# miniufo/xinvert

Measured on AMD Instinct MI355X. Metric: SOR grid-points*iters/sec (fp64) at 3600x1800, masked points counted, higher is better.
Workload: dtype f64

## Files before the change

### xinvert_amd/csrc/xinv_pipe2d.h

```cpp
#pragma once
#include "xinv_fused.h"

#define XINV_PIPE_P 4
#ifndef XINV_PIPE_B
#define XINV_PIPE_B 2
#endif
#define XINV_PIPE_LAG (XINV_PIPE_B + 5)
#define XINV_PIPE_NS 4
#define XINV_PIPE_UW(np) (128 * (np) - 4 * XINV_PIPE_P)
#ifndef XINV_PIPE_PF0
#define XINV_PIPE_PF0 4
#endif
#ifndef XINV_PIPE_PF
#define XINV_PIPE_PF 4
#endif

template <class M, unsigned UM> struct PipeRec {
    static constexpr int NCO = M::NC - 1;
    static constexpr int NUNI = __builtin_popcount(UM & ((1u << NCO) - 1u));
    static constexpr bool HOIST = M::template hoist<UM>();
    static constexpr int NW = NUNI + (HOIST ? 2 : 0);
    static constexpr int RW = NW == 0 ? 0 : (NW <= 4 ? 4 : 8);
};

struct RowFactorArgs {
    const double *c[5];
    int64_t sc[5];
    int64_t yc, xc;
    int gen;
    unsigned um;
    int hoist, rw;
    XinvScal sc_;
    double *rowf;
};

#ifdef XINV_AUX_KERNELS
__global__ __launch_bounds__(256) void k_row_factor(RowFactorArgs a)
{
    const int64_t j = (int64_t)blockIdx.x * 256 + threadIdx.x, m = blockIdx.y;
    if (j >= a.yc) return;
    const double u = a.sc_.undef;
    const bool inner = (j >= 1 && j <= a.yc - 2);
    const int nco = a.gen ? 5 : 2;
    const double ones = __longlong_as_double(-1LL);
    double *f = a.rowf + (m * a.yc + j) * a.rw;
    double v[5];
    int k = 0;
    bool def = true;
    for (int q = 0; q < nco; q++) {
        v[q] = 0.0;
        if ((a.um >> q) & 1u) { v[q] = a.c[q][m * a.sc[q] + j * a.xc]; f[k++] = v[q]; def = def && (v[q] != u); }
    }
    if (a.hoist) {
        double rq = 0.0, rok = 0.0;
        if (inner) {
            if (!a.gen) {
                const double aP = a.c[0][m * a.sc[0] + (j + 1) * a.xc], a0 = v[0], c = v[1];
                rq = a.sc_.optArg / ((aP + a0) * a.sc_.ratioSqr + (c + c));
                rok = (def && (aP != u)) ? ones : 0.0;
            } else {
                const double A = v[0], C = v[1], F = v[4];
                rq = a.sc_.optArg / ((A * a.sc_.ratioSqr + C) * 2.0
                                     - F * a.sc_.delxSqr);
                rok = def ? ones : 0.0;
            }
        }
        f[k++] = rq; f[k++] = rok;
    }
    for (; k < a.rw; k++) f[k] = 0.0;
}
#endif

struct PointFactorArgs {
    const double *c[6];
    int64_t sc[6];
    int64_t yc, xc, n;
    XinvScal sc_;
    double *q;
    int *flag;
};
#ifdef XINV_AUX_KERNELS
__global__ __launch_bounds__(256) void k_point_factor(PointFactorArgs a)
{
    const int64_t m = blockIdx.y;
    const double u = a.sc_.undef;
    bool zero = false, differ = false;
    for (int64_t t = (int64_t)blockIdx.x * 256 + threadIdx.x; t < a.n; t += (int64_t)gridDim.x * 256) {
        const int64_t j = t / a.xc;
        const double A = a.c[0][m * a.sc[0] + t], C = a.c[1][m * a.sc[1] + t], Dd = a.c[2][m * a.sc[2] + t];
        const double E = a.c[3][m * a.sc[3] + t], F = a.c[4][m * a.sc[4] + t], G = a.c[5][m * a.sc[5] + t];
        differ = differ || (__double_as_longlong(A) != __double_as_longlong(C));
        const bool ok = (j >= 1) && (j <= a.yc - 2) && (G != u) && (A != u) && (C != u) && (Dd != u) && (E != u) && (F != u);
        double q = 0.0;
        if (ok) {
            q = a.sc_.optArg / ((A * a.sc_.ratioSqr + C) * 2.0
                                - F * a.sc_.delxSqr);
            zero = zero || (q == 0.0);
        }
        a.q[m * a.n + t] = q;
    }
    if (__any(zero) && (threadIdx.x & 63) == 0) atomicOr(a.flag, 1);
    if (__any(differ) && (threadIdx.x & 63) == 0) atomicOr(a.flag, 2);
}
#endif

__device__ __forceinline__ void xinv_pipe_barrier()
{
    asm volatile("s_waitcnt lgkmcnt(0)\n\ts_barrier" ::: "memory");
}

typedef const double __attribute__((address_space(4))) *xinv_cdouble_ptr;
typedef const char __attribute__((address_space(1))) *xinv_gcptr;
typedef char __attribute__((address_space(1))) *xinv_gptr;
typedef double xinv_v2d __attribute__((ext_vector_type(2)));
typedef const xinv_v2d __attribute__((address_space(1))) *xinv_gcd2ptr;
typedef const double __attribute__((address_space(1))) *xinv_gcdptr;
typedef xinv_v2d __attribute__((address_space(1))) *xinv_gd2ptr;
typedef double __attribute__((address_space(1))) *xinv_gdptr;

__device__ __forceinline__ void pipe_extend_fix(double2 &edge, const double2 &inner, double inner_w,
                                                const LaneCols &lc, bool tall, double u)
{
    if (lc.cls_x == 1) { if (inner.x != u) edge.x = inner.x; }
    else if (lc.cls_x == 2) { if (inner.y != u) edge.x = inner.y; }
    else if (lc.cls_x == 3) {
        if (tall && inner.x != u) edge.x = inner.x;
        if (inner_w != u) edge.x = inner_w;
    }
    if (lc.cls_y == 1) { if (inner.y != u) edge.y = inner.y; }
    else if (lc.cls_y == 3) {
        if (tall && inner.y != u) edge.y = inner.y;
        if (inner.x != u) edge.y = inner.x;
    }
}

template <class M, unsigned UM, bool FR, int NP, bool AL, bool EXT, int PW, int PF, bool SEAM = false>
__device__ __forceinline__ void xinv_pipe_wave(const FusedArgs &a, int64_t m, int yu0, int yu1,
                                               const LaneCols (&lc)[NP], const int64_t (&st0)[NP], int lane,
                                               double2 (*ring)[XINV_PIPE_NS][NP * (FR ? 2 : 1)][XINV_WAVE], int gtot,
                                               double &acc, int &cnt,
                                               unsigned long long seam_lanes = 0ull)
{
    constexpr int P = XINV_PIPE_P, H = 2 * P, D = 4, LAG = XINV_PIPE_LAG, B = XINV_PIPE_B;
    constexpr int R = PF + D;
    constexpr int PFR = M::PIPE_PFR;
    using REC = PipeRec<M, UM>;
    constexpr int NC = M::NC, FQ = M::NC - 1, RW = REC::RW;
    constexpr bool HOIST = REC::HOIST;
    constexpr int RS = FR ? 2 : 1;
    static_assert(R % D == 0 && R % B == 0 && R % XINV_PIPE_NS == 0,
                  "the unroll period must keep row parity, ring slots and barriers compile-time");
    const int ycr = (int)a.yc;
    const unsigned rowbytes = (unsigned)a.xc * 8u;
    const double u = a.sc_.undef;
    const int slice_bytes = (int)(rowbytes * (unsigned)ycr);
    const __amdgpu_buffer_rsrc_t rsS = __builtin_amdgcn_make_buffer_rsrc((void *)(a.src + m * a.sS), 0, slice_bytes, 0x00020000);
    const __amdgpu_buffer_rsrc_t rsD = __builtin_amdgcn_make_buffer_rsrc((void *)(a.dst + m * a.sS), 0, slice_bytes, 0x00020000);
    __amdgpu_buffer_rsrc_t rsC[NC];
#pragma unroll
    for (int q = 0; q < NC; q++)
        rsC[q] = __builtin_amdgcn_make_buffer_rsrc((void *)(a.c[q] + m * a.sc[q]), 0, slice_bytes, 0x00020000);
    const xinv_cdouble_ptr rowf = (xinv_cdouble_ptr)(uintptr_t)(reinterpret_cast<const double *>(a.rowf) + m * a.yc * RW);
    unsigned lo0[NP], lo1[NP], so0[NP], so1[NP];
#pragma unroll
    for (int q = 0; q < NP; q++) {
        lo0[q] = (unsigned)lc[q].l0 * 8u; lo1[q] = (unsigned)lc[q].l1 * 8u;
        so0[q] = lc[q].use_x ? (unsigned)st0[q] * 8u : 0xffffffffu;
        so1[q] = lc[q].use_y ? (unsigned)(st0[q] + 1) * 8u : 0xffffffffu;
    }

    unsigned long long okx64[NP], oky64[NP];
    double nsx[NP], nsy[NP];
    int nnx[NP], nny[NP];
#pragma unroll
    for (int q = 0; q < NP; q++) {
        okx64[q] = __builtin_amdgcn_ballot_w64(lc[q].ok_x) & ~seam_lanes; oky64[q] = __builtin_amdgcn_ballot_w64(lc[q].ok_y);
        nsx[q] = nsy[q] = 0.0; nnx[q] = nny[q] = 0;
    }
    static_assert(!SEAM || (NP == 1 && !AL && PipeRec<M, UM>::HOIST),
                  "seam variants: one column pair per lane, per-row records, updates under EXEC masks");

    const int in_lo = yu0 - H + 2 * PW;
    const int in_hi = yu1 - 1 + H - 2 * PW;

    double2 sw[NP][R];
    CoefWin<NC, R> cw[NP];
    double rokw[R];
#pragma unroll
    for (int t = 0; t < R; t++) {
        rokw[t] = 0.0;
#pragma unroll
        for (int q = 0; q < NP; q++) {
            sw[q][t] = make_double2(0.0, 0.0);
            cw[q].rq[t] = 0.0; cw[q].mx[t] = 0u; cw[q].my[t] = 0u;
#pragma unroll
            for (int c = 0; c < NC; c++) { cw[q].v[c][t] = make_double2(0.0, 0.0); cw[q].s[c][t] = 0.0; }
        }
    }

    const int maxo = (int)(rowbytes * (unsigned)(ycr - 1));
    int nxo = (yu0 - H + 2 * PW) * (int)rowbytes;
    int nxr = (yu0 - H + 2 * PW) * (RW * 8);
    auto ldrow = [&](__amdgpu_buffer_rsrc_t rs, int soff, auto qtag) {
        constexpr int q = decltype(qtag)::value;
        double2 v;
        if (AL) {
            const auto t = __builtin_amdgcn_raw_buffer_load_b128(rs, (int)lo0[q], soff, 0);
            v.x = __hiloint2double((int)t[1], (int)t[0]); v.y = __hiloint2double((int)t[3], (int)t[2]);
        } else {
            const auto t0 = __builtin_amdgcn_raw_buffer_load_b64(rs, (int)lo0[q], soff, 0);
            const auto t1 = __builtin_amdgcn_raw_buffer_load_b64(rs, (int)lo1[q], soff, 0);
            v.x = __hiloint2double((int)t0[1], (int)t0[0]); v.y = __hiloint2double((int)t1[1], (int)t1[0]);
        }
        return v;
    };
    auto request = [&](int, auto stag) {
        constexpr int slot = decltype(stag)::value;
        const int soff = min(max(nxo, 0), maxo);
        nxo += (int)rowbytes;
        asm("" : "+s"(nxo));
        xinv_unroll_steps([&](auto qtag) {
            constexpr int q = decltype(qtag)::value;
            if (PW == 0) sw[q][slot] = ldrow(rsS, soff, qtag);
            xinv_unroll_steps([&](auto ctag) {
                constexpr int c = decltype(ctag)::value;
                if (!((UM >> c) & 1u) && !(FR && c == FQ && PW > 0)) cw[q].v[c][slot] = ldrow(rsC[c], soff, qtag);
            }, std::make_integer_sequence<int, NC>{});
        }, std::make_integer_sequence<int, NP>{});
    };
    auto request_rf = [&](int, auto stag) {
        constexpr int slot = decltype(stag)::value;
        if constexpr (RW > 0) {
            const unsigned roff = (unsigned)min(max(nxr, 0), (ycr - 1) * (RW * 8));
            nxr += RW * 8;
            const xinv_cdouble_ptr pr = (xinv_cdouble_ptr)((const char __attribute__((address_space(4))) *)rowf + roff);
            double rec[RW];
#pragma unroll
            for (int k = 0; k < RW; k++) rec[k] = pr[k];
#pragma unroll
            for (int q = 0; q < NP; q++) {
                int k = 0;
#pragma unroll
                for (int c = 0; c < NC - 1; c++)
                    if ((UM >> c) & 1u) cw[q].s[c][slot] = rec[k++];
                if (HOIST) { cw[q].rq[slot] = rec[k]; rokw[slot] = rec[k + 1]; }
            }
        }
    };
    xinv_unroll_steps([&](auto ttag) { request(in_lo + decltype(ttag)::value, ttag); asm volatile("" ::: "memory"); },
                      std::make_integer_sequence<int, PF>{});
    xinv_unroll_steps([&](auto ttag) { request_rf(in_lo + decltype(ttag)::value, ttag); },
                      std::make_integer_sequence<int, PFR>{});

    auto half_pass = [&](auto xtag, auto jtag, auto ptag, auto mtag, auto fixt) {
        constexpr int X = decltype(xtag)::value, sj = decltype(jtag)::value, sjp = decltype(ptag)::value,
                      sjm = decltype(mtag)::value;
        constexpr bool FIX = decltype(fixt)::value;
        static_assert(!FIX || (X == 0 && NP == 1), "column xc-1 sits in an .x slot");
        const double edge = (X == 0) ? xinv_lane_up(sw[NP - 1][sj].y) : xinv_lane_down(sw[0][sj].x);
        double nv[NP];
#pragma unroll
        for (int q = 0; q < NP; q++) {
            double w, e;
            if (X == 0) { w = (q == 0) ? edge : sw[q > 0 ? q - 1 : 0][sj].y; e = sw[q][sj].y; }
            else        { w = sw[q][sj].x; e = (q == NP - 1) ? edge : sw[q < NP - 1 ? q + 1 : q][sj].x; }
            if constexpr (FIX) e = xinv_lane_down(sw[q][sj].x);
            const double t = M::template inc<X, UM, R, false>(cw[q], sj, sjp, comp<X>(sw[q][sj]), comp<X>(sw[q][sjp]),
                                              comp<X>(sw[q][sjm]), w, e, a.sc_);
            if constexpr (HOIST) {
                const unsigned long long rm = (FIX ? seam_lanes : (X ? oky64[q] : okx64[q])) &
                                              (unsigned long long)__double_as_longlong(rokw[sj]);
                if constexpr (ModelFma<M>::value)
                    nv[q] = xinv_fma_where_ne(comp<X>(sw[q][sj]), t, cw[q].rq[sj], comp<X>(cw[q].v[FQ][sj]), u, rm);
                else
                    nv[q] = xinv_add_where_ne(comp<X>(sw[q][sj]), t, comp<X>(cw[q].v[FQ][sj]), u, rm);
            } else {
                const unsigned long long pm = __builtin_amdgcn_ballot_w64((X ? cw[q].my[sj] : cw[q].mx[sj]) != 0u);
                nv[q] = xinv_add_where(comp<X>(sw[q][sj]), t, pm);
            }
        }
#pragma unroll
        for (int q = 0; q < NP; q++) setc<X>(sw[q][sj], nv[q]);
    };
    auto half_sweep = [&](auto xtag, auto jtag, auto ptag, auto mtag) {
        constexpr int X = decltype(xtag)::value;
        half_pass(xtag, jtag, ptag, mtag, std::false_type{});
        if constexpr (SEAM && X == 0) {
            constexpr int sj = decltype(jtag)::value;
            half_pass(xtag, jtag, ptag, mtag, std::true_type{});
            sw[0][sj].y = xinv_bitsel64(seam_lanes, sw[0][sj].x, sw[0][sj].y);
        }
    };

    int g = 0;
#pragma unroll
    for (; g < LAG * PW; g++) {
        if (PW > 0 && g == LAG * PW - 1) {
#pragma unroll
            for (int q = 0; q < NP; q++) {
                sw[q][0] = ring[PW - 1][(2 * PW) % XINV_PIPE_NS][q * RS][lane];
                if (FR) cw[q].v[FQ][0] = ring[PW - 1][(2 * PW) % XINV_PIPE_NS][q * RS + 1][lane];
            }
        }
        if ((g + 1) % B == 0) xinv_pipe_barrier();
    }

    for (int rb_ = in_lo; rb_ <= in_hi; rb_ += R) {
        xinv_unroll_steps([&](auto utag) {
            constexpr int U = decltype(utag)::value;
            constexpr int X = (U & 1) ? 0 : 1;
#define SLOT(w) ((U - (w) + 4 * R) % R)
#define RSLOT(w) ((2 * PW + U - (w) + 64 * XINV_PIPE_NS) % XINV_PIPE_NS)
#define ITAG(v) std::integral_constant<int, (v)>{}
            const int r = rb_ + U;
            request(r + PF, ITAG((U + PF) % R));
            request_rf(r + PFR, ITAG((U + PFR) % R));
            if (PW > 0) {
#pragma unroll
                for (int q = 0; q < NP; q++) {
                    sw[q][(U + 1) % R] = ring[PW - 1][RSLOT(-1)][q * RS][lane];
                    if (FR) cw[q].v[FQ][(U + 1) % R] = ring[PW - 1][RSLOT(-1)][q * RS + 1][lane];
                }
            }
            if constexpr (!HOIST) {
                const bool rv = (r - 1 >= 1) && (r - 1 <= ycr - 2);
#pragma unroll
                for (int q = 0; q < NP; q++)
                    M::template derive<UM, R, false>(cw[q], SLOT(0), SLOT(1), rv && lc[q].ok_x, rv && lc[q].ok_y, a.sc_);
            }
            {
                const int ja = r - 1;
                constexpr int sj = SLOT(1), sjp = SLOT(0), sjm = SLOT(2);
                if (EXT) {
                    if (ja == 1 || ja == ycr - 2) {
                        const double wl = xinv_lane_up(sw[NP - 1][sj].y);
#pragma unroll
                        for (int q = 0; q < NP; q++) {
                            const double iw = (q == 0) ? wl : sw[q > 0 ? q - 1 : 0][sj].y;
                            if (ja == 1) pipe_extend_fix(sw[q][sjm], sw[q][sj], iw, lc[q], a.tall, u);
                            if (ja == ycr - 2) pipe_extend_fix(sw[q][sjp], sw[q][sj], iw, lc[q], a.tall, u);
                        }
                    }
                }
                half_sweep(ITAG(X), ITAG(sj), ITAG(sjp), ITAG(sjm));
            }
            {
                const int jb = r - 2;
                constexpr int sj = SLOT(2), sjp = SLOT(1), sjm = SLOT(3);
                half_sweep(ITAG(X), ITAG(sj), ITAG(sjp), ITAG(sjm));
                if ((unsigned)(jb - yu0) < (unsigned)(yu1 - yu0)) {
#pragma unroll
                    for (int q = 0; q < NP; q++) {
                        const double2 t = sw[q][sj];
                        xinv_norm_row(nsx[q], nsy[q], nnx[q], nny[q], t.x, t.y, u);
                    }
                }
                if (PW < P - 1) {
#pragma unroll
                    for (int q = 0; q < NP; q++) {
                        ring[PW][RSLOT(2)][q * RS][lane] = sw[q][sj];
                        if (FR) ring[PW][RSLOT(2)][q * RS + 1][lane] = cw[q].v[FQ][sj];
                    }
                } else if ((unsigned)(jb - yu0) < (unsigned)(yu1 - yu0)) {
                    const int doff = jb * (int)rowbytes;
                    xinv_unroll_steps([&](auto qtag) {
                        constexpr int q = decltype(qtag)::value;
                        const double2 t = sw[q][sj];
                        typedef unsigned xinv_v4u __attribute__((__vector_size__(16)));
                        typedef unsigned xinv_v2u __attribute__((__vector_size__(8)));
                        if (AL) {
                            const xinv_v4u tv = {(unsigned)__double2loint(t.x), (unsigned)__double2hiint(t.x),
                                                 (unsigned)__double2loint(t.y), (unsigned)__double2hiint(t.y)};
                            __builtin_amdgcn_raw_buffer_store_b128(tv, rsD, (int)so0[q], doff, 0);
                        } else {
                            const xinv_v2u tx = {(unsigned)__double2loint(t.x), (unsigned)__double2hiint(t.x)};
                            const xinv_v2u ty = {(unsigned)__double2loint(t.y), (unsigned)__double2hiint(t.y)};
                            __builtin_amdgcn_raw_buffer_store_b64(tx, rsD, (int)so0[q], doff, 0);
                            __builtin_amdgcn_raw_buffer_store_b64(ty, rsD, (int)so1[q], doff, 0);
                        }
                    }, std::make_integer_sequence<int, NP>{});
                }
            }
            if ((LAG * PW + U + 1) % B == 0) xinv_pipe_barrier();
#undef SLOT
#undef RSLOT
#undef ITAG
        }, std::make_integer_sequence<int, R>{});
        g += R;
    }
    for (; g < gtot; g++) if ((g + 1) % B == 0) xinv_pipe_barrier();
#pragma unroll
    for (int q = 0; q < NP; q++) {
        acc += (lc[q].use_x ? nsx[q] : 0.0);
        acc += (lc[q].use_y ? nsy[q] : 0.0);
        cnt += (lc[q].use_x ? nnx[q] : 0) + (lc[q].use_y ? nny[q] : 0);
    }
}

template <class M, unsigned UM, bool FR, int NP, bool AL, bool EXT, bool SEAM = false>
__global__ __launch_bounds__(64 * XINV_PIPE_P) void k_pipe2d(FusedArgs a_)
{
    xinv_fresh_scalar_cache();
    constexpr int P = XINV_PIPE_P, K = P, H = 2 * K, LAG = XINV_PIPE_LAG, B = XINV_PIPE_B;
    __shared__ double2 ring[P - 1][XINV_PIPE_NS][NP * (FR ? 2 : 1)][XINV_WAVE];

    unsigned tag;
    int T;
    double acc = 0.0;
    int cnt = 0;
    const int wave = threadIdx.x >> 6, lane = threadIdx.x & 63;
    int pwi;
    {
    const FusedArgs &a = a_;
    const int64_t m = a.member0 + blockIdx.y;
    XinvCtl *ctl = a.ctl + m;
    if (!a.force && xinv_ctl_done(ctl)) return;
    if (a.lag && (int)blockIdx.x == a.nwg) { xinv_lag_reduce_prev(a, ctl, m); return; }
    tag = a.lag ? a.tag : xinv_ctl_seq(ctl);

    const int NB = a.nwg;
    {
        const int L = blockIdx.x, q = NB >> 3, rem = NB & 7, xcd = L & 7, idx = L >> 3;
        T = xcd * q + (xcd < rem ? xcd : rem) + idx;
    }
    pwi = (wave + (int)(blockIdx.x >> 8)) & (P - 1);
    int wt = T;
    bool active = wt < a.nstrip * a.nrb;
    if constexpr (SEAM) {
        if (!a.tile_list && NB == a.nstrip * a.nrb)
            wt = xinv_seam_tile(xinv_heavy_first((int)blockIdx.x, NB, (a.nstrip == 1 ? 1 : 2) * a.nrb), a.nstrip, a.nrb);
    }
    if (a.tile_list) {
        wt = a.tile_list[m * a.ntl + T];
        active = wt >= 0;
        wt = active ? wt : 0;
    }
    int rb = wt / a.nstrip, strip = wt - rb * a.nstrip;
    const int64_t xc = a.xc, yc = a.yc;
    int yu0, yu1;
    if (a.RY > 0) {
        yu0 = rb * a.RY;
        yu1 = (yu0 + a.RY < (int)yc) ? yu0 + a.RY : (int)yc;
    } else {
        yu0 = (int)((((int64_t)rb * yc) / a.nrb) & ~(int64_t)1);
        yu1 = (rb + 1 == a.nrb) ? (int)yc : (int)((((int64_t)(rb + 1) * yc) / a.nrb) & ~(int64_t)1);
    }
    const int UW = SEAM ? xinv_ring_uw(xc, H) : XINV_PIPE_UW(NP), HW = SEAM ? xinv_ring_hw(xc, H, strip) : H;
    const int64_t xu0 = (int64_t)strip * UW;
    LaneCols lc[NP];
    int64_t st0[NP];
    RingSeam rs = {0ull, false};
#pragma unroll
    for (int q = 0; q < NP; q++) {
        if constexpr (SEAM) lc[q] = make_lanecols_ring(xu0, HW, UW, lane, xc, rs);
        else lc[q] = make_lanecols<AL>(xu0, H, UW, lane, xc, a.per != 0, NP, q);
        st0[q] = xu0 - HW + 2 * NP * lane + 2 * q;
    }

    if (active) {
        const int ry = yu1 - yu0;
        int gtot = 0;
#pragma unroll
        for (int pw = 0; pw < P; pw++) {
            const int per = (pw == 0 ? XINV_PIPE_PF0 : XINV_PIPE_PF) + 4;
            const int n = ry + 2 * H - 4 * pw;
            const int g = LAG * pw + ((n + per - 1) / per) * per;
            gtot = g > gtot ? g : gtot;
        }
        gtot = ((gtot + B - 1) / B) * B;
        const bool wraps = rs.any;
#define XINV_PIPE_MARCH(SM) \
        switch (pwi) { \
        case 0: xinv_pipe_wave<M, UM, FR, NP, AL, EXT, 0, XINV_PIPE_PF0, SM>(a, m, yu0, yu1, lc, st0, lane, ring, gtot, acc, cnt, rs.lanes); break; \
        case 1: xinv_pipe_wave<M, UM, FR, NP, AL, EXT, 1, XINV_PIPE_PF, SM>(a, m, yu0, yu1, lc, st0, lane, ring, gtot, acc, cnt, rs.lanes); break; \
        case 2: xinv_pipe_wave<M, UM, FR, NP, AL, EXT, 2, XINV_PIPE_PF, SM>(a, m, yu0, yu1, lc, st0, lane, ring, gtot, acc, cnt, rs.lanes); break; \
        default: xinv_pipe_wave<M, UM, FR, NP, AL, EXT, 3, XINV_PIPE_PF, SM>(a, m, yu0, yu1, lc, st0, lane, ring, gtot, acc, cnt, rs.lanes); break; \
        }
        if (wraps) { XINV_PIPE_MARCH(SEAM) } else { XINV_PIPE_MARCH(false) }
#undef XINV_PIPE_MARCH
    }
    }
    const FusedArgs __attribute__((address_space(4))) *kp =
        (const FusedArgs __attribute__((address_space(4))) *)__builtin_amdgcn_kernarg_segment_ptr();
    asm volatile("" : "+s"(kp) :: "memory");
    if (kp->no_ctl) return;
    const int64_t m = kp->member0 + blockIdx.y;
    XinvCtl *ctl = kp->ctl + m;
    const int NB = kp->nwg;
    struct { unsigned long long *psum; const double *xsum; const long long *xcnt; int lag; XinvStop stop; const void *hook; } a;
    a.psum = kp->psum; a.xsum = kp->xsum; a.xcnt = kp->xcnt; a.lag = kp->lag;
    a.hook = XINV_TEST_HOOKS ? (const void *)kp->dbg : nullptr;
    a.stop.mxLoop = kp->stop.mxLoop; a.stop.tolerance = kp->stop.tolerance;
    a.stop.stop_on_zero_norm = kp->stop.stop_on_zero_norm;

    {
        unsigned long long *pw = a.psum + (size_t)m * XINV_KMAX * NB * XINV_PW;
        const double ws = xinv_wave_sum(acc);
        const long long wc = xinv_wave_sum_ll((long long)cnt);
        if (lane == 0 && !xinv_hook_withhold(a.hook, T, tag, m)) {
            const unsigned long long hi = (unsigned long long)tag << 32;
            const unsigned long long bits = (unsigned long long)__double_as_longlong(ws);
            unsigned long long *q = pw + ((size_t)pwi * NB + T) * XINV_PW;
            __hip_atomic_store(q + 0, hi | (bits & 0xffffffffull), __ATOMIC_RELAXED, __HIP_MEMORY_SCOPE_AGENT);
            __hip_atomic_store(q + 1, hi | (bits >> 32), __ATOMIC_RELAXED, __HIP_MEMORY_SCOPE_AGENT);
            __hip_atomic_store(q + 2, hi | (unsigned long long)(unsigned)wc, __ATOMIC_RELAXED,
                               __HIP_MEMORY_SCOPE_AGENT);
        }
        if (a.lag || blockIdx.x != gridDim.x - 1) return;
        __syncthreads();
        xinv_norm_reduce<K, P>(wave, lane, NB, tag, pw, ctl, a.stop, a.xsum ? a.xsum[m] : 0.0,
                               a.xcnt ? a.xcnt[m] : 0);
    }
}
```

### xinvert_amd/csrc/xinv_tiles.h

```cpp
#pragma once
#include <cstdint>
#ifndef __HIPCC__
#ifndef __host__
#define __host__
#endif
#ifndef __device__
#define __device__
#endif
#endif

struct TileRows { int strip; int64_t y0, y1; };
__host__ __device__ inline TileRows xinv_tile_rows(int wt, int nstrip, int nrb, int64_t yc, int RY)
{
    TileRows t;
    const int rb = wt / nstrip;
    t.strip = wt - rb * nstrip;
    if (RY > 0) { t.y0 = (int64_t)rb * RY; t.y1 = (t.y0 + RY < yc) ? t.y0 + RY : yc; }
    else {
        t.y0 = (((int64_t)rb * yc) / nrb) & ~(int64_t)1;
        t.y1 = (rb + 1 == nrb) ? yc : ((((int64_t)(rb + 1) * yc) / nrb) & ~(int64_t)1);
    }
    return t;
}

__host__ __device__ inline int xinv_heavy_first(int L, int n, int nh)
{
    const int hq = (nh < n ? nh : n) >> 3, xcd = L & 7, idx = L >> 3;
    if (idx < hq) return idx * 8 + xcd;
    const int nr = n - 8 * hq, q = nr >> 3, rem = nr & 7;
    return 8 * hq + xcd * q + (xcd < rem ? xcd : rem) + (idx - hq);
}
__host__ __device__ inline int xinv_seam_tile(int s, int nstrip, int nrb)
{
    const int edges = nstrip == 1 ? 1 : 2, nh = edges * nrb;
    if (s < nh) {
        const int e = s / nrb, rb = s - e * nrb;
        return rb * nstrip + (e == 0 ? nstrip - 1 : 0);
    }
    const int k = s - nh, nl = nstrip > edges ? nstrip - edges : 1, rb = k / nl;
    return rb * nstrip + (k - rb * nl) + 1;
}

__host__ __device__ inline bool xinv_ring_asym(int64_t xc, int H) { return xc >= (int64_t)(128 - 2 * H - 2) + H; }
__host__ __device__ inline int xinv_ring_uw(int64_t xc, int H) { return 128 - 2 * H - (xinv_ring_asym(xc, H) ? 2 : 4); }
__host__ __device__ inline int xinv_ring_hw(int64_t xc, int H, int strip)
{
    return xinv_ring_asym(xc, H) ? (strip == 0 ? H + 2 : H) : H + 2;
}

__host__ __device__ inline int xinv_p3_slot_tile(int L, int nfull, int nkc, int &kc)
{
    int g;
    kc = 0;
    if (L < nfull) g = L;
    else { const int q = L - nfull; g = nfull + q / nkc; kc = q - (g - nfull) * nkc; }
    return g;
}
__host__ __device__ inline bool xinv_p3_slot_reduces(int L, int nfull, int nkc, int NT, int ml)
{
    const int gl = (ml + 1) * NT - 1;
    return (gl < nfull) ? (L == gl) : (L == nfull + (gl - nfull) * nkc + nkc - 1);
}
__host__ __device__ inline int xinv_p3_slot_member_tile(int L, int nfull, int NT, int ml, int g)
{
    if (L < nfull) {
        const int L0 = ml * NT;
        const int n = (L0 + NT <= nfull) ? NT : (nfull - L0);
        const int xcd = L & 7;
        auto below = [](int e, int x) { return (e >> 3) * x + ((e & 7) < x ? (e & 7) : x); };
        auto same = [](int e, int x) { return e <= x ? 0 : ((e - x + 7) >> 3); };
        return (below(L0 + n, xcd) - below(L0, xcd)) + (same(L, xcd) - same(L0, xcd));
    }
    return g - ml * NT;
}
struct P3Slot { int ml, Tj, kc; bool whole, reducer; };
__host__ __device__ inline P3Slot xinv_p3_slot(int L, int nfull, int nkc, int NT)
{
    P3Slot s;
    s.whole = L < nfull;
    const int g = xinv_p3_slot_tile(L, nfull, nkc, s.kc);
    s.ml = g / NT;
    s.reducer = xinv_p3_slot_reduces(L, nfull, nkc, NT, s.ml);
    s.Tj = xinv_p3_slot_member_tile(L, nfull, NT, s.ml, g);
    return s;
}

__host__ inline int64_t xinv_p3_whole_tiles(int64_t tiles, int nk, int64_t KC, int64_t zc, int cus_, double *cost_out = nullptr)
{
    const bool no_rem = cus_ < 0;
    const int64_t cus = cus_ < 0 ? -cus_ : cus_;
    auto cdiv64 = [](int64_t a, int64_t b) { return (a + b - 1) / b; };
    const double cf = (double)(zc + 4), cs = (double)(KC + 14);
    double best = (double)cdiv64(tiles, cus) * cf;
    int64_t nfull = tiles;
    if (nk > 1) {
        const double call = (double)cdiv64(tiles * nk, cus) * cs;
        if (call < best * 0.97) { best = call; nfull = 0; }
        const int64_t r = tiles % cus, R = tiles / cus;
        if (r && R && !no_rem) {
            const double crem = (double)R * cf + (double)cdiv64(r * nk, cus) * cs;
            if (crem < best * 0.985) { best = crem; nfull = tiles - r; }
        }
    }
    if (cost_out) *cost_out = best;
    return nfull;
}

__host__ __device__ inline bool xinv_p3_extend_ok(int64_t yc, int joff, int RJ, int H, int RR)
{
    if ((H + joff) % RR == RR - 1) return false;
    const int64_t jbo = (yc - 1 + joff) / RJ;
    auto together = [&](int64_t jb) { return ((yc - 2) - (jb * RJ - H - joff)) % RR != RR - 1; };
    if (!together(jbo)) return false;
    if (jbo > 0 && (yc - 1 + joff) - jbo * RJ <= 1 && !together(jbo - 1)) return false;
    return true;
}
__host__ __device__ inline int xinv_p3_extend_joff(int64_t yc, int RJ, int H, int RR)
{
    return xinv_p3_extend_ok(yc, 0, RJ, H, RR) ? 0 : (xinv_p3_extend_ok(yc, 2, RJ, H, RR) ? 2 : -1);
}

__host__ inline int64_t xinv_cdiv(int64_t a, int64_t b) { return (a + b - 1) / b; }

__host__ inline double xinv_tile_cost(int64_t wgs, int64_t rows, int K, int occ, int occ_cap, double lone, int pipe_lag)
{
    const bool pipe = pipe_lag > 0;
    occ = occ < occ_cap ? occ : occ_cap;
    occ = occ > 1 ? occ : 1;
    const int64_t cap = 256 * (int64_t)occ, period = pipe ? 4 : 2 * K + 2;
    const int64_t steps = pipe ? xinv_cdiv(rows + 1 + 4 + 3 * pipe_lag, 8) * 8
                               : xinv_cdiv(rows + 1 + 4 * K, period) * period;
    const int64_t r = xinv_cdiv(wgs, cap), rounds = r > 1 ? r : 1;
    const int64_t w_last = wgs - (rounds - 1) * cap;
    const double full = pipe ? 1.5 + occ : ((occ == 1) ? lone : (double)occ);
    const double last = pipe ? 1.5 + (double)xinv_cdiv(w_last, 256) : ((w_last <= 256) ? lone : (double)xinv_cdiv(w_last, 256));
    return ((double)(rounds - 1) * full + last) * (double)steps;
}

__host__ inline int64_t xinv_choose_row_blocks(int64_t yc, int64_t nstrip, int64_t nbatch, int K, int occ, int occ_cap,
                                               double lone, int pipe_lag)
{
    const bool pipe = pipe_lag > 0;
    int64_t best = 1; double best_cost = 1e300;
    const int64_t n0 = xinv_cdiv(yc, pipe ? 512 : 128), nmin = n0 > 1 ? n0 : 1, nmax = nmin > yc / 4 ? nmin : yc / 4;
    for (int64_t nr = nmin; nr <= nmax; nr++) {
        const int64_t wgs = xinv_cdiv(nstrip * nr, pipe ? 1 : 4) * nbatch;
        const double cost = xinv_tile_cost(wgs, xinv_cdiv(yc, nr), K, occ, occ_cap, lone, pipe_lag);
        if (cost <= best_cost * 1.0001) { best_cost = cost < best_cost ? cost : best_cost; best = nr; }
    }
    return best;
}

__host__ inline int64_t xinv_k_chunk_planes(int64_t zc, int nk) { return xinv_cdiv(xinv_cdiv(zc, nk), 4) * 4; }
template <class Cost>
__host__ inline int xinv_choose_k_chunks(int64_t zc, Cost cost)
{
    int best = 1; double best_cost = 1e300;
    for (int nk = 1; nk <= 16; nk++) {
        const int64_t KC = xinv_k_chunk_planes(zc, nk);
        if (nk > 1 && (KC < 16 || (int64_t)(nk - 1) * KC >= zc)) break;
        const double c = cost(nk, KC);
        if (c < best_cost * 0.97) { best_cost = c; best = nk; }
    }
    return best;
}
__host__ inline int xinv_k_chunks_fused3d(int64_t zc, int64_t wgs)
{
    return xinv_choose_k_chunks(zc, [&](int nk, int64_t KC) { return (double)xinv_cdiv(wgs * nk, 256) * (double)(KC + (nk > 1 ? 10 : 2)); });
}
__host__ inline int xinv_k_chunks_pipe3d(int64_t zc, int64_t tiles, int cus)
{
    return xinv_choose_k_chunks(zc, [&](int nk, int64_t KC) { double c; xinv_p3_whole_tiles(tiles, nk, KC, zc, cus, &c); return c; });
}
```

Baseline: 730.7 billion.

## Start later pipeline wavefronts earlier when their padded step count leaves slack

Adds a schedule helper that, for each wavefront after the first, shifts its row march four steps earlier when rounding its row count up to the step period leaves at least four idle steps. The shifted wavefront starts prefetching and sweeping sooner, so the total step count (gtot) and the trailing idle barriers can shrink. The cost is more complex start-up logic that must keep ring slots, colour parity and barrier positions in step, enforced by static asserts. It also hardcodes four wavefronts and a halo of 8.

New measurement: 733.3 billion (median of 6 runs). Within noise of the previous version (+0.4%).

```diff
diff --git a/xinvert_amd/csrc/xinv_pipe2d.h b/xinvert_amd/csrc/xinv_pipe2d.h
--- a/xinvert_amd/csrc/xinv_pipe2d.h
+++ b/xinvert_amd/csrc/xinv_pipe2d.h
@@ -182,6 +182,7 @@
 
     const int in_lo = yu0 - H + 2 * PW;
     const int in_hi = yu1 - 1 + H - 2 * PW;
+    const int front = PW > 0 ? xinv_pipe_sched(yu1 - yu0, PW, XINV_PIPE_PF0, XINV_PIPE_PF, LAG, B).front : 0;
 
     double2 sw[NP][R];
     CoefWin<NC, R> cw[NP];
@@ -199,8 +200,8 @@
     }
 
     const int maxo = (int)(rowbytes * (unsigned)(ycr - 1));
-    int nxo = (yu0 - H + 2 * PW) * (int)rowbytes;
-    int nxr = (yu0 - H + 2 * PW) * (RW * 8);
+    int nxo = (in_lo - front) * (int)rowbytes;
+    int nxr = (in_lo - front) * (RW * 8);
     auto ldrow = [&](__amdgpu_buffer_rsrc_t rs, int soff, auto qtag) {
         constexpr int q = decltype(qtag)::value;
         double2 v;
@@ -247,9 +248,9 @@
             }
         }
     };
-    xinv_unroll_steps([&](auto ttag) { request(in_lo + decltype(ttag)::value, ttag); asm volatile("" ::: "memory"); },
+    xinv_unroll_steps([&](auto ttag) { request(in_lo - front + decltype(ttag)::value, ttag); asm volatile("" ::: "memory"); },
                       std::make_integer_sequence<int, PF>{});
-    xinv_unroll_steps([&](auto ttag) { request_rf(in_lo + decltype(ttag)::value, ttag); },
+    xinv_unroll_steps([&](auto ttag) { request_rf(in_lo - front + decltype(ttag)::value, ttag); },
                       std::make_integer_sequence<int, PFR>{});
 
     auto half_pass = [&](auto xtag, auto jtag, auto ptag, auto mtag, auto fixt) {
@@ -292,20 +293,29 @@
         }
     };
 
+    constexpr int FRONT = PW > 0 ? 4 : 0;
+    static_assert(FRONT <= LAG * PW && FRONT % XINV_PIPE_NS == 0 && FRONT % 2 == 0 && FRONT % B == 0,
+                  "a shifted march keeps ring slots, colour parity and barrier positions in step with the row");
     int g = 0;
 #pragma unroll
-    for (; g < LAG * PW; g++) {
-        if (PW > 0 && g == LAG * PW - 1) {
-#pragma unroll
-            for (int q = 0; q < NP; q++) {
-                sw[q][0] = ring[PW - 1][(2 * PW) % XINV_PIPE_NS][q * RS][lane];
-                if (FR) cw[q].v[FQ][0] = ring[PW - 1][(2 * PW) % XINV_PIPE_NS][q * RS + 1][lane];
-            }
-        }
+    for (; g < LAG * PW - FRONT; g++)
         if ((g + 1) % B == 0) xinv_pipe_barrier();
-    }
-
-    for (int rb_ = in_lo; rb_ <= in_hi; rb_ += R) {
+    if (PW > 0 && front == 0) {
+#pragma unroll
+        for (int t = LAG * PW - FRONT; t < LAG * PW; t++) {
+            if (t == LAG * PW - 1) {
+#pragma unroll
+                for (int q = 0; q < NP; q++) {
+                    sw[q][0] = ring[PW - 1][(2 * PW) % XINV_PIPE_NS][q * RS][lane];
+                    if (FR) cw[q].v[FQ][0] = ring[PW - 1][(2 * PW) % XINV_PIPE_NS][q * RS + 1][lane];
+                }
+            }
+            if ((t + 1) % B == 0) xinv_pipe_barrier();
+        }
+        g = LAG * PW;
+    }
+
+    for (int rb_ = in_lo - front; rb_ <= in_hi; rb_ += R) {
         xinv_unroll_steps([&](auto utag) {
             constexpr int U = decltype(utag)::value;
             constexpr int X = (U & 1) ? 0 : 1;
@@ -458,16 +468,8 @@
     }
 
     if (active) {
-        const int ry = yu1 - yu0;
-        int gtot = 0;
-#pragma unroll
-        for (int pw = 0; pw < P; pw++) {
-            const int per = (pw == 0 ? XINV_PIPE_PF0 : XINV_PIPE_PF) + 4;
-            const int n = ry + 2 * H - 4 * pw;
-            const int g = LAG * pw + ((n + per - 1) / per) * per;
-            gtot = g > gtot ? g : gtot;
-        }
-        gtot = ((gtot + B - 1) / B) * B;
+        static_assert(P == 4 && H == 8, "xinv_pipe_sched: four wavefronts, 16 - 4 pw halo rows");
+        const int gtot = xinv_pipe_sched(yu1 - yu0, 0, XINV_PIPE_PF0, XINV_PIPE_PF, LAG, B).gtot;
         const bool wraps = rs.any;
 #define XINV_PIPE_MARCH(SM) \
         switch (pwi) { \
diff --git a/xinvert_amd/csrc/xinv_tiles.h b/xinvert_amd/csrc/xinv_tiles.h
--- a/xinvert_amd/csrc/xinv_tiles.h
+++ b/xinvert_amd/csrc/xinv_tiles.h
@@ -46,6 +46,24 @@
 __host__ __device__ inline int xinv_ring_hw(int64_t xc, int H, int strip)
 {
     return xinv_ring_asym(xc, H) ? (strip == 0 ? H + 2 : H) : H + 2;
+}
+
+struct PipeSched { int front, g0, steps, gtot; };
+__host__ __device__ inline PipeSched xinv_pipe_sched(int ry, int pw, int PF0, int PF, int LAG, int B)
+{
+    PipeSched s = {0, 0, 0, 0};
+    int last = 0;
+    for (int w = 0; w < 4; w++) {
+        const int per = (w == 0 ? PF0 : PF) + 4;
+        const int n = ry + 16 - 4 * w;
+        const int steps = ((n + per - 1) / per) * per;
+        const int front = (w > 0 && steps - n >= 4) ? 4 : 0;
+        const int g0 = LAG * w - front;
+        if (w == pw) { s.front = front; s.g0 = g0; s.steps = steps; }
+        last = g0 + steps > last ? g0 + steps : last;
+    }
+    s.gtot = ((last + B - 1) / B) * B;
+    return s;
 }
 
 __host__ __device__ inline int xinv_p3_slot_tile(int L, int nfull, int nkc, int &kc)
```
